# TencentYoutuResearch/NeRF-Loc

Measured on AMD Instinct MI355X. Metric: rendered rays/sec (4096 rays×128 samples, 256-wide MLP) at 1/2/4/8 MI355X, higher is better.
Workload: dtype f16mx (neural-point kernel, conv_out and feat_mlp.0: fp16 hi.hi + two MX-FP6 cross terms, 1.5 MFMA-equivalents per product; every other GEMM 3-term split-bf16 or split-fp16; fp32 accumulate; meets 1e-4)

## Files before the change

### nerf_loc_amd/csrc/hier.hip

```cpp
#include "mvdec.h"

namespace {
using namespace nlmv;

struct QueryCam { float w2c[12]; float kinv[9]; };

__global__ __launch_bounds__(256) void coarse_view_kernel(const NlViews vw, const QueryCam qc, const float* __restrict__ visf,
                                                          const float* __restrict__ dw, const float* __restrict__ pix ,
                                                          const float* __restrict__ zc , int R, int Sc,
                                                          float* __restrict__ alpha_out , float* __restrict__ vis_out,
                                                          float* __restrict__ mask_out) {
  const int i = blockIdx.x * blockDim.x + threadIdx.x;
  const int v = blockIdx.y;
  if (i >= R * Sc) return;
  const int r = i / Sc, s = i - r * Sc;
  const float u = pix[2 * r], vv = pix[2 * r + 1];
  const float* K = qc.kinv;
  const float c0 = K[0] * u + K[1] * vv + K[2], c1 = K[3] * u + K[4] * vv + K[5], c2 = K[6] * u + K[7] * vv + K[8];
  const float* Wm = qc.w2c;
  const float t0 = Wm[3], t1 = Wm[7], t2 = Wm[11];
  float cen[3], dir[3];
#pragma unroll
  for (int a = 0; a < 3; ++a) {
    const float r0 = Wm[a], r1 = Wm[4 + a], r2 = Wm[8 + a];
// ... 112 lines not shown
    al = al * (1.f - inv) + inv * -15.f;
    a = nl_sigmoid(al);
  }
  float inc = on ? 1.f - a : 1.f;
#pragma unroll
  for (int o = 1; o < 64; o <<= 1) {
    float t = __shfl_up(inc, o, 64);
    if (lane >= o) inc *= t;
  }
  float T = __shfl_up(inc, 1, 64);
  if (lane == 0) T = 1.f;
  const float w = on ? a * T : 0.f;
  if (on) weights[(size_t)r * Sc + lane] = w;
  const float d = wave_sum(on ? w * zc[(size_t)r * Sc + lane] : 0.f);
  if (lane == 0 && depth_coarse) depth_coarse[r] = d;
}

__global__ __launch_bounds__(256) void sample_pdf_kernel(const float* __restrict__ zc, const float* __restrict__ wc, int Sc,
                                                         const float* __restrict__ u, int Ni, const float* __restrict__ zb, int Sb,
                                                         int R, float* __restrict__ z_out) {
  __shared__ float s_cdf[4][64];
  __shared__ float s_bins[4][64];
  __shared__ float s_sort[4][256];
  const int lane = threadIdx.x & 63, wv = threadIdx.x >> 6;
  const int r = blockIdx.x * 4 + wv;
  if (r >= R) return;
  const int nb = Sc - 2;
  const float eps = 1e-5f;
  float wgt = (lane < nb) ? wc[(size_t)r * Sc + 1 + lane] + eps : 0.f;
  const float tot = wave_sum(wgt);
  const float pdf = wgt / tot;
  s_bins[wv][lane] = (lane < Sc - 1) ? 0.5f * (zc[(size_t)r * Sc + lane] + zc[(size_t)r * Sc + lane + 1]) : 0.f;
  s_cdf[wv][lane] = pdf;
  __builtin_amdgcn_wave_barrier();
  if (lane == 0) {
    float run = 0.f;
    float prev = 0.f;
    for (int i = 0; i < nb; ++i) { const float p = s_cdf[wv][i]; s_cdf[wv][i] = prev; run += p; prev = run; }
    s_cdf[wv][nb] = prev;
  }
  __builtin_amdgcn_wave_barrier();
  const int S = Sb + Ni;
  for (int i = lane; i < 256; i += 64) s_sort[wv][i] = i < Sb ? zb[(size_t)r * Sb + i] : 3.4e38f;
  for (int i = lane; i < Ni; i += 64) {
    const float uu = u[(size_t)r * Ni + i];
    int lo = 0, hi = nb + 1;
    while (lo < hi) { const int mid = (lo + hi) >> 1; if (s_cdf[wv][mid] > uu) hi = mid; else lo = mid + 1; }
    const int below = lo - 1 < 0 ? 0 : lo - 1;
    const int above = lo > nb ? nb : lo;
    const float c0 = s_cdf[wv][below], c1 = s_cdf[wv][above];
    const float b0 = s_bins[wv][below], b1 = s_bins[wv][above];
    float den = c1 - c0;
    if (den < eps) den = 1.f;
    s_sort[wv][Sb + i] = b0 + (uu - c0) / den * (b1 - b0);
  }
  __builtin_amdgcn_wave_barrier();
  for (int k = 2; k <= 256; k <<= 1) {
    for (int j = k >> 1; j > 0; j >>= 1) {
#pragma unroll
      for (int e = 0; e < 2; ++e) {
        const int t = lane + 64 * e;
        const int i = 2 * j * (t / j) + (t % j);
        const int p = i + j;
        const bool up = ((i & k) == 0);
        const float x = s_sort[wv][i], y = s_sort[wv][p];
        if ((x > y) == up) { s_sort[wv][i] = y; s_sort[wv][p] = x; }
      }
      __builtin_amdgcn_wave_barrier();
    }
  }
  for (int i = lane; i < S; i += 64) z_out[(size_t)r * S + i] = s_sort[wv][i];
}

}

int nl_launch_coarse_weights(const NlViews& vw, const float* w2c_kinv_host, const float* visf_hwc, const float* dec_w, const void* dpack,
                             int precision, const float* pix, const float* zc, int64_t R, int Sc, float* ws_alpha, float* ws_vis, float* ws_mask,
                             float* weights, float* depth_coarse, hipStream_t st) {
  if (R <= 0) return NL_OK;
  if (Sc < 3 || Sc > 64) return NL_ERR_UNSUPPORTED;
  QueryCam qc;
  for (int i = 0; i < 12; ++i) qc.w2c[i] = w2c_kinv_host[i];
  for (int i = 0; i < 9; ++i) qc.kinv[i] = w2c_kinv_host[12 + i];
  if (precision == NL_PREC_F32 || R * Sc > 0x7fffffffll / 32) {
    dim3 grid((unsigned)nl_cdiv(R * Sc, 256), (unsigned)vw.V);
    hipLaunchKernelGGL(coarse_view_kernel, grid, dim3(256), 0, st, vw, qc, visf_hwc, dec_w, pix, zc, (int)R, Sc, ws_alpha, ws_vis, ws_mask);
  } else {
    const int tpv = (int)nl_cdiv(R * Sc, 32), total = tpv * vw.V;
    const int blocks = (int)(nl_cdiv(total, 4) < 2048 ? nl_cdiv(total, 4) : 2048);
    hipLaunchKernelGGL(coarse_view_mfma_kernel<true>, dim3(blocks), dim3(256), 0, st, vw, qc, visf_hwc, (const uint4*)dpack, pix, zc, (int)R, Sc, tpv,
                       total, ws_alpha, ws_vis, ws_mask);
  }
  hipLaunchKernelGGL(coarse_ray_kernel, dim3((unsigned)nl_cdiv(R, 4)), dim3(256), 0, st, ws_alpha, ws_vis, ws_mask, zc, vw.V, (int)R, Sc,
                     weights, depth_coarse);
  NL_LAUNCH_CHECK();
  return NL_OK;
}

int nl_launch_sample_pdf(const float* zc, const float* wc, int Sc, const float* u, int Ni, const float* zb, int Sb, int64_t R,
                         float* z_out, hipStream_t st) {
  if (R <= 0) return NL_OK;
  if (Sc < 3 || Sc > 64 || Sb + Ni > 256 || Ni < 1) return NL_ERR_UNSUPPORTED;
  hipLaunchKernelGGL(sample_pdf_kernel, dim3((unsigned)nl_cdiv(R, 4)), dim3(256), 0, st, zc, wc, Sc, u, Ni, zb, Sb, (int)R, z_out);
  NL_LAUNCH_CHECK();
  return NL_OK;
}
```

### nerf_loc_amd/csrc/mvagg.hip

```cpp
#include "mvdec.h"

namespace {
using namespace nlmv;

__global__ void chw_to_hwc_kernel(const float* __restrict__ src, float* __restrict__ dst, int V, int Cc, int HW) {
  size_t i = (size_t)blockIdx.x * blockDim.x + threadIdx.x;
  size_t total = (size_t)V * Cc * HW;
  if (i >= total) return;
  int c = (int)(i % Cc);
  size_t t = i / Cc;
  int p = (int)(t % HW);
  int v = (int)(t / HW);
  dst[i] = src[((size_t)v * Cc + c) * HW + p];
}

__global__ __launch_bounds__(256) void mv_vis_kernel(const NlViews vw, const float* __restrict__ visf ,
                                                     const float* __restrict__ dw, const float* __restrict__ xyz, int N,
                                                     float* __restrict__ vis_out , float* __restrict__ dd_out ) {
  const int n = blockIdx.x * blockDim.x + threadIdx.x;
  const int v = blockIdx.y;
  if (n >= N) return;
  const float X = xyz[3 * (size_t)n], Y = xyz[3 * (size_t)n + 1], Z = xyz[3 * (size_t)n + 2];
  float px, py, depth;
  const bool valid = project_neuray(vw.P2[v], X, Y, Z, vw.Wimg, vw.H, px, py, depth);
  float x[32];
  sample_visf(visf + (size_t)v * vw.vh * vw.vw * 32, vw.vh, vw.vw, vw.Wimg, vw.H, px, py, valid, x);
  float m0, m1, v0, v1, aw, vs;
  decode_all(dw, x, m0, m1, v0, v1, vs, aw);

  const float ni = -1.f / vw.near_, fi = -1.f / vw.far_;
  float refd = -1.f / (m0 * (fi - ni) + ni);
  refd = fminf(fmaxf(refd, vw.near_), vw.far_);
  const float dd = fabsf(depth - refd) / (vw.far_ - vw.near_);
  const float dn = (-1.f / fmaxf(depth, 1e-5f) - ni) / (fi - ni);
  const float c0 = (0.5f + 0.5f * tanhf((dn - m0) * v0)) * vs;
  const float c1 = (0.5f + 0.5f * tanhf((dn - m1) * v1)) * vs;
  float vis = (1.f - c0) * aw + (1.f - c1) * (1.f - aw);
  vis = valid ? vis : 0.f;
  vis_out[(size_t)v * N + n] = vis;
  dd_out[(size_t)v * N + n] = dd;
}

template <bool X3>
__global__ __launch_bounds__(256) void mv_vis_mfma_kernel(const NlViews vw, const float* __restrict__ visf ,
                                                          const uint4* __restrict__ dpack, const float* __restrict__ xyz, int N,
                                                          int tiles_per_view, int total_tiles, float* __restrict__ vis_out,
                                                          float* __restrict__ dd_out) {
  __shared__ uint4 sw[MVD_LDS_UINT4];
  const int tid = threadIdx.x, lane = tid & 63, wave = tid >> 6;
  const int hh = lane >> 5, j = lane & 31;
  if (X3) __builtin_amdgcn_s_setreg(1473, 1);
  mvd_load_lds<X3>(sw, dpack, tid, 256);
  __syncthreads();

  for (int tile = blockIdx.x * 4 + wave; tile < total_tiles; tile += gridDim.x * 4) {
    const int v = __builtin_amdgcn_readfirstlane(tile / tiles_per_view);
    const int n = (tile - v * tiles_per_view) * 32 + j;
    const bool live = n < N;
    const int nn = live ? n : N - 1;
    const float X = xyz[3 * (size_t)nn], Y = xyz[3 * (size_t)nn + 1], Z = xyz[3 * (size_t)nn + 2];
    float px, py, depth;
    const bool valid = project_neuray(vw.P2[v], X, Y, Z, vw.Wimg, vw.H, px, py, depth);
    if (__ballot(valid && live) == 0ull) {
      if (live && hh == 0) {
        vis_out[(size_t)v * N + n] = 0.f;
        dd_out[(size_t)v * N + n] = 0.f;
      }
      continue;
    }
    float x0[8], x1[8];
    mvd_tap16(visf + (size_t)v * vw.vh * vw.vw * 32 + 8 * hh, vw.vh, vw.vw, vw.Wimg, vw.H, px, py, valid, x0, x1);
    float m0, m1, v0, v1, aw, vs;
    mvd_decode_tile<X3>(sw, lane, x0, x1, m0, m1, v0, v1, vs, aw);
    const float ni = -1.f / vw.near_, fi = -1.f / vw.far_;
    float refd = -1.f / (m0 * (fi - ni) + ni);
    refd = fminf(fmaxf(refd, vw.near_), vw.far_);
    const float dd = fabsf(depth - refd) / (vw.far_ - vw.near_);
    const float dn = (-1.f / fmaxf(depth, 1e-5f) - ni) / (fi - ni);
    const float c0 = (0.5f + 0.5f * tanhf((dn - m0) * v0)) * vs;
    const float c1 = (0.5f + 0.5f * tanhf((dn - m1) * v1)) * vs;
    float vis = (1.f - c0) * aw + (1.f - c1) * (1.f - aw);
    vis = valid ? vis : 0.f;
    if (live && hh == 0) {
      vis_out[(size_t)v * N + n] = vis;
      dd_out[(size_t)v * N + n] = dd;
    }
  }
}

__global__ void pack_mv_decoder_kernel(const float* __restrict__ dec , uint4* __restrict__ out) {
  unsigned short* o16 = reinterpret_cast<unsigned short*>(out);
  unsigned short* h16 = reinterpret_cast<unsigned short*>(out + MVD_F16);
  float* of = reinterpret_cast<float*>(out + MVD_F32);
  const int i = blockIdx.x * blockDim.x + threadIdx.x;
  auto f2bf = [](float x) { unsigned int u = __float_as_uint(x); u += 0x7fffu + ((u >> 16) & 1u); return (unsigned short)(u >> 16); };
  auto f2h = [](float x) { const _Float16 h = (_Float16)x; return __builtin_bit_cast(unsigned short, h); };
  auto h2f = [](unsigned short b) { return (float)__builtin_bit_cast(_Float16, b); };
  if (i < 4096) {
    const int t = i & 7, lane = (i >> 3) & 63, d = (i >> 9) & 3, q = i >> 11;
    const float v = dec[d * DEC_STRIDE + (lane & 31) * 32 + 16 * q + 8 * (lane >> 5) + t];
    const unsigned short h = f2bf(v);
    o16[(size_t)MVD_W1 * 8 + i] = h;
    o16[(size_t)(MVD_W1 + 512) * 8 + i] = f2bf(v - __uint_as_float(((unsigned)h) << 16));
    const unsigned short g = f2h(v);
    h16[(size_t)MVD_W1 * 8 + i] = g;
    h16[(size_t)(MVD_W1 + 512) * 8 + i] = f2h(v - h2f(g));
  } else if (i < 8192) {
    const int e = i - 4096;
    const int t = e & 7, lane = (e >> 3) & 63, s = (e >> 9) & 1, d = e >> 10;
    const int fin = 16 * s + (t & 3) + 8 * (t >> 2) + 4 * (lane >> 5);
    const float v = dec[d * DEC_STRIDE + 1056 + (lane & 31) * 32 + fin];
    const unsigned short h = f2bf(v);
    o16[(size_t)MVD_W2 * 8 + e] = h;
    o16[(size_t)(MVD_W2 + 512) * 8 + e] = f2bf(v - __uint_as_float(((unsigned)h) << 16));
    const unsigned short g = f2h(v);
    h16[(size_t)MVD_W2 * 8 + e] = g;
    h16[(size_t)(MVD_W2 + 512) * 8 + e] = f2h(v - h2f(g));
  } else if (i < 8192 + 128) { const int e = i - 8192; of[e] = dec[(e >> 5) * DEC_STRIDE + 1024 + (e & 31)]; }
  else if (i < 8192 + 256) { const int e = i - 8192 - 128; of[128 + e] = dec[(e >> 5) * DEC_STRIDE + 2080 + (e & 31)]; }
  else if (i < 8192 + 512) {
    const int e = i - 8192 - 256;
    const int r = e & 15, hh = (e >> 4) & 1, u = (e >> 5) & 1, d = e >> 6;
    const int idx = (r & 3) + 8 * (r >> 2) + 4 * hh;
    of[256 + e] = dec[d * DEC_STRIDE + 2112 + u * 32 + idx];
  } else if (i < 8192 + 520) { const int e = i - 8192 - 512; of[512 + e] = dec[(e >> 1) * DEC_STRIDE + 2176 + (e & 1)]; }
  if (i < 8192) {
    unsigned short* t16 = reinterpret_cast<unsigned short*>(out + MVD_T);
    const int which = i >> 12, e = i & 4095;
    const int t = e & 7, lane = (e >> 3) & 63, s = (e >> 9) & 1, d = e >> 10;
    const int u = 16 * s + (t & 3) + 8 * (t >> 2) + 4 * (lane >> 5);
    const int row = lane & 31;
    float v;
    if (which == 0) v = dec[d * DEC_STRIDE + 1056 + u * 32 + row];
    else {
      const int hh = (row >> 2) & 1, r = (row & 3) + 4 * (row >> 3);
      const int chan = r < 8 ? 8 * hh + r : 16 + 8 * hh + (r - 8);
      v = dec[d * DEC_STRIDE + u * 32 + chan];
    }
    const unsigned short h = f2bf(v);
    t16[(size_t)which * 1024 * 8 + e] = h;
    t16[(size_t)which * 1024 * 8 + 512 * 8 + e] = f2bf(v - __uint_as_float(((unsigned)h) << 16));
  }
}

__device__ __forceinline__ float rl(float v, int lane) { return __int_as_float(__builtin_amdgcn_readlane(__float_as_int(v), lane)); }
__device__ __forceinline__ int rli(int v, int lane) { return __builtin_amdgcn_readlane(v, lane); }

template <int VT, bool V4, bool EXACT>
__global__ __launch_bounds__(256, VT <= 4 ? 4 : (VT <= 10 ? 3 : 2)) void mv_stats_kernel(const NlViews vw, const float* __restrict__ viewsdev ,
                                                       const float* __restrict__ images ,
                                                       const float* __restrict__ feat , int C,
                                                       const float* __restrict__ xyz, int N,
                                                       const float* __restrict__ vis_in, const float* __restrict__ dd_in,
                                                       float* __restrict__ g393, int ldg, float* __restrict__ rgb_feat ,
                                                       float* __restrict__ vis_ang , int* __restrict__ valid_s,
                                                       const float* __restrict__ pfeat ,
                                                       const float* __restrict__ blw ,
                                                       float* __restrict__ bl1 , float* __restrict__ rgbv ) {
  const int lane = threadIdx.x & 63;
  const int n = nl_xcd_block() * 4 + (threadIdx.x >> 6);
  if (n >= N) return;
  const int V = EXACT ? VT : vw.V;
  const float X = xyz[3 * (size_t)n], Y = xyz[3 * (size_t)n + 1], Z = xyz[3 * (size_t)n + 2];
  const int F = C + 3;

  const int vl = lane < V ? lane : 0;
// ... 357 lines not shown
    Tap4 cur = issue(0);
#pragma unroll
    for (int v = 0; v < VT; ++v) {
      if (v < V) {
        Tap4 nxt = cur;
        if (v + 1 < VT && v + 1 < V) nxt = issue(v + 1);
        if (!active(v)) {
          if (live) {
            *(float4*)(bl1 + ((size_t)n * V + v) * 32 + 4 * j) = make_float4(0.f, 0.f, 0.f, 0.f);
            if (j == 0) *(float4*)(rgbv + ((size_t)n * V + v) * 4) = make_float4(slot0[v * MS8_SLOT + 17], slot0[v * MS8_SLOT + 18], slot0[v * MS8_SLOT + 19], 0.f);
          }
          cur = nxt;
          continue;
        }
        const float* sl = slot0 + v * MS8_SLOT;
        const float4 w = *(const float4*)(sl + 2), ang = *(const float4*)(sl + 10);
        const float s_vis = sl[14], r = sl[17], gg = sl[18], b = sl[19];
        const float pv[4] = {fmaf(cur.t[3].x, w.w, fmaf(cur.t[2].x, w.z, fmaf(cur.t[1].x, w.y, cur.t[0].x * w.x))),
                             fmaf(cur.t[3].y, w.w, fmaf(cur.t[2].y, w.z, fmaf(cur.t[1].y, w.y, cur.t[0].y * w.x))),
                             fmaf(cur.t[3].z, w.w, fmaf(cur.t[2].z, w.z, fmaf(cur.t[1].z, w.y, cur.t[0].z * w.x))),
                             fmaf(cur.t[3].w, w.w, fmaf(cur.t[2].w, w.z, fmaf(cur.t[1].w, w.y, cur.t[0].w * w.x)))};
        float o[4];
#pragma unroll
        for (int c = 0; c < 4; ++c) {
          float a = pv[c] + bb[c];
          a = fmaf(bw[c][0], r, a); a = fmaf(bw[c][1], gg, a); a = fmaf(bw[c][2], b, a);
          a = fmaf(bw[c][3], s_vis, a);
          a = fmaf(bw[c][4], ang.x, a); a = fmaf(bw[c][5], ang.y, a); a = fmaf(bw[c][6], ang.z, a); a = fmaf(bw[c][7], ang.w, a);
          o[c] = a;
        }
        if (live) {
          *(float4*)(bl1 + ((size_t)n * V + v) * 32 + 4 * j) = make_float4(o[0], o[1], o[2], o[3]);
          if (j == 0) *(float4*)(rgbv + ((size_t)n * V + v) * 4) = make_float4(r, gg, b, s_vis);
        }
        cur = nxt;
      }
    }
  }

  if (live && j == 0) {
    float mean = 0.f, wsum = 0.f;
#pragma unroll
    for (int v = 0; v < VT; ++v) { if (v < V) { mean += slot0[v * MS8_SLOT + 15] * wg[v]; wsum += wg[v]; } }
    float var = 0.f;
#pragma unroll
    for (int v = 0; v < VT; ++v) { if (v < V) { const float d = slot0[v * MS8_SLOT + 15] - mean; var += wg[v] * (d * d); } }
    g[2 * F] = mean;
    g[2 * F + 1] = var;
    g[2 * F + 2] = wsum / (float)V;
    for (int p = 2 * F + 3; p < ldg; ++p) g[p] = 0.f;
    valid_s[n] = cnt1 > 1 ? 1 : 0;
  }
}

}

int nl_launch_chw_to_hwc(const float* src, float* dst, int V, int Cc, int HW, hipStream_t st) {
  size_t total = (size_t)V * Cc * HW;
  hipLaunchKernelGGL(chw_to_hwc_kernel, dim3((unsigned)nl_cdiv(total, 256)), dim3(256), 0, st, src, dst, V, Cc, HW);
  NL_LAUNCH_CHECK();
  return NL_OK;
}

int nl_launch_mv_vis(const NlViews& vw, const float* visf_hwc, const float* dec_w, const float* xyz, int64_t N,
                     float* vis_out, float* dd_out, hipStream_t st) {
  if (N <= 0) return NL_OK;
  dim3 grid((unsigned)nl_cdiv(N, 256), (unsigned)vw.V);
  hipLaunchKernelGGL(mv_vis_kernel, grid, dim3(256), 0, st, vw, visf_hwc, dec_w, xyz, (int)N, vis_out, dd_out);
  NL_LAUNCH_CHECK();
  return NL_OK;
}

size_t nl_mv_decoder_pack_bytes() { return (size_t)MVD_PACK_UINT4 * 16; }

int nl_pack_mv_decoder(const float* dec_valu_layout, void* out, hipStream_t st) {
  hipLaunchKernelGGL(pack_mv_decoder_kernel, dim3((8192 + 520 + 255) / 256), dim3(256), 0, st, dec_valu_layout, (uint4*)out);
  NL_LAUNCH_CHECK();
  return NL_OK;
}

int nl_launch_mv_vis_mfma(const NlViews& vw, const float* visf_hwc, const void* dpack, const float* xyz, int64_t N, float* vis_out,
                          float* dd_out, bool x3, hipStream_t st) {
  if (N <= 0) return NL_OK;
  const int tpv = (int)nl_cdiv(N, 32), total = tpv * vw.V;
  constexpr int64_t max_blocks = 2048;
  const int blocks = (int)(nl_cdiv(total, 4) < max_blocks ? nl_cdiv(total, 4) : max_blocks);
  if (x3) hipLaunchKernelGGL(mv_vis_mfma_kernel<true>, dim3(blocks), dim3(256), 0, st, vw, visf_hwc, (const uint4*)dpack, xyz, (int)N, tpv, total, vis_out, dd_out);
  else hipLaunchKernelGGL(mv_vis_mfma_kernel<false>, dim3(blocks), dim3(256), 0, st, vw, visf_hwc, (const uint4*)dpack, xyz, (int)N, tpv, total, vis_out, dd_out);
  NL_LAUNCH_CHECK();
  return NL_OK;
}

int nl_launch_mv_stats(const NlViews& vw, const float* viewsdev, const float* images, const float* feat, int C, const float* xyz, int64_t N,
                       const float* vis_in, const float* dd_in, float* g393, int ldg, float* rgb_feat, float* vis_ang,
                       int* valid_s, const float* pfeat, const float* blw, float* bl1, float* rgbv, hipStream_t st) {
  if (N <= 0) return NL_OK;
  if (C > 192) return NL_ERR_UNSUPPORTED;
  const bool v4 = (C % 4 == 0) && ((((size_t)feat) & 15) == 0);
  if (v4 && !rgb_feat && !vis_ang) {
    dim3 grid8(nl_xcd_grid(nl_cdiv(N, 32)));
#define NL_MS8(VT) hipLaunchKernelGGL((mv_stats8_kernel<VT>), grid8, dim3(256), sizeof(float) * 4 * 8 * VT * MS8_SLOT, st, vw, viewsdev, images, feat, C, \
                                      xyz, (int)N, vis_in, dd_in, g393, ldg, valid_s, pfeat, blw, bl1, rgbv)
    if (vw.V <= 4) NL_MS8(4); else if (vw.V <= 8) NL_MS8(8); else if (vw.V <= 10) NL_MS8(10); else NL_MS8(16);
#undef NL_MS8
    NL_LAUNCH_CHECK();
    return NL_OK;
  }
  dim3 grid(nl_xcd_grid(nl_cdiv(N, 4)));
  const bool ex = vw.V == 4 || vw.V == 8 || vw.V == 10 || vw.V == 16;
#define NL_MS1(VT, V4, EX)                                                                                                              \
  hipLaunchKernelGGL((mv_stats_kernel<VT, V4, EX>), grid, dim3(256), 0, st, vw, viewsdev, images, feat, C, xyz, (int)N, vis_in, dd_in, \
                     g393, ldg, rgb_feat, vis_ang, valid_s, pfeat, blw, bl1, rgbv)
#define NL_MS1_BUCKET(VT)                 \
  do {                                    \
    if (v4 && ex) NL_MS1(VT, true, true); \
    else if (v4) NL_MS1(VT, true, false); \
    else NL_MS1(VT, false, false);        \
  } while (0)
  if (vw.V <= 4) NL_MS1_BUCKET(4);
  else if (vw.V <= 8) NL_MS1_BUCKET(8);
  else if (vw.V <= 10) NL_MS1_BUCKET(10);
  else NL_MS1_BUCKET(16);
#undef NL_MS1_BUCKET
#undef NL_MS1
  NL_LAUNCH_CHECK();
  return NL_OK;
}
```

### nerf_loc_amd/csrc/mvdec.h

```cpp
#pragma once
#include "common.h"

namespace nlmv {

struct Taps {
  int x0, y0;
  float nw, ne, sw, se;
  bool mw, me, mn, ms;
};

template <bool ALIGN, bool BORDER>
__device__ __forceinline__ Taps make_taps(float xn, float yn, int Wm, int Hm) {
  float ix, iy;
  if (ALIGN) {
    ix = (xn + 1.f) * ((float)(Wm - 1) / 2.f);
    iy = (yn + 1.f) * ((float)(Hm - 1) / 2.f);
  } else {
    ix = (xn + 1.f) * ((float)Wm / 2.f) - 0.5f;
    iy = (yn + 1.f) * ((float)Hm / 2.f) - 0.5f;
  }
  if (BORDER) {
    ix = fminf((float)(Wm - 1), fmaxf(ix, 0.f));
    iy = fminf((float)(Hm - 1), fmaxf(iy, 0.f));
  }
// ... 44 lines not shown
  const float* w4 = w2 + 1024 + 32;
  float a0 = w4[64], a1 = w4[65];
#pragma unroll
  for (int i = 0; i < 32; ++i) {
    a0 = fmaf(w4[i], h2[i], a0);
    a1 = fmaf(w4[32 + i], h2[i], a1);
  }
  o0 = a0;
  o1 = a1;
}


__device__ __forceinline__ bool project_neuray(const float* P, float X, float Y, float Z, int Wimg, int H, float& px, float& py, float& depth) {
  const float cx = fmaf(P[2], Z, fmaf(P[1], Y, P[0] * X)) + P[3];
  const float cy = fmaf(P[6], Z, fmaf(P[5], Y, P[4] * X)) + P[7];
  depth = fmaf(P[10], Z, fmaf(P[9], Y, P[8] * X)) + P[11];
  const bool bad = fabsf(depth) < 1e-4f;
  if (bad) depth = 1e-3f;
  px = cx / depth; py = cy / depth;
  const bool outside = (px < -0.5f) | (px >= (float)Wimg - 0.5f) | (py < -0.5f) | (py >= (float)H - 0.5f);
  return !bad && !outside;
}

__device__ __forceinline__ void sample_visf(const float* __restrict__ base, int h, int w, int Wimg, int H, float px, float py, bool valid, float (&x)[32]) {
  if (valid) {
    const float xn = px / (float)(Wimg - 1) * 2.f - 1.f;
    const float yn = py / (float)(H - 1) * 2.f - 1.f;
    const Taps t = make_taps<false, true>(xn, yn, w, h);
    const int xe = t.x0 + 1, ys = t.y0 + 1;
#pragma unroll
    for (int c4 = 0; c4 < 8; ++c4) {
      float4 a = make_float4(0, 0, 0, 0), b = a, c = a, d = a;
      if (t.mn && t.mw) a = *(const float4*)(base + ((size_t)t.y0 * w + t.x0) * 32 + c4 * 4);
      if (t.mn && t.me) b = *(const float4*)(base + ((size_t)t.y0 * w + xe) * 32 + c4 * 4);
      if (t.ms && t.mw) c = *(const float4*)(base + ((size_t)ys * w + t.x0) * 32 + c4 * 4);
      if (t.ms && t.me) d = *(const float4*)(base + ((size_t)ys * w + xe) * 32 + c4 * 4);
      x[c4 * 4 + 0] = a.x * t.nw + b.x * t.ne + c.x * t.sw + d.x * t.se;
      x[c4 * 4 + 1] = a.y * t.nw + b.y * t.ne + c.y * t.sw + d.y * t.se;
      x[c4 * 4 + 2] = a.z * t.nw + b.z * t.ne + c.z * t.sw + d.z * t.se;
      x[c4 * 4 + 3] = a.w * t.nw + b.w * t.ne + c.w * t.sw + d.w * t.se;
    }
  } else {
#pragma unroll
    for (int i = 0; i < 32; ++i) x[i] = 0.f;
  }
}

__device__ __forceinline__ void decode_all(const float* __restrict__ dw, const float (&x)[32], float& m0, float& m1, float& v0, float& v1, float& vs, float& aw) {
  float dummy;
  decoder(dw + 0 * DEC_STRIDE, x, m0, m1);
  decoder(dw + 1 * DEC_STRIDE, x, v0, v1);
  decoder(dw + 2 * DEC_STRIDE, x, aw, dummy);
  decoder(dw + 3 * DEC_STRIDE, x, vs, dummy);
  m0 = nl_softplus(m0); m1 = nl_softplus(m1);
  v0 = nl_softplus(v0) + 0.05f; v1 = nl_softplus(v1) + 0.05f;
  aw = nl_sigmoid(aw); vs = nl_sigmoid(vs);
}

typedef __bf16 mvd_bf16x8 __attribute__((ext_vector_type(8)));
typedef _Float16 mvd_f16x8 __attribute__((ext_vector_type(8)));
typedef float mvd_f32x16 __attribute__((ext_vector_type(16)));

constexpr int MVD_W1 = 0;
constexpr int MVD_W2 = 1024;
constexpr int MVD_F32 = 2048;
constexpr int MVD_NF32 = (128 + 128 + 256 + 8) / 4;
constexpr int MVD_F16 = MVD_F32 + MVD_NF32;
constexpr int MVD_T = MVD_F16 + 2048;
constexpr int MVD_PACK_UINT4 = MVD_T + 2048;
constexpr int MVD_LDS_UINT4 = 2048 + MVD_NF32;

template <bool X3>
__device__ __forceinline__ void mvd_load_lds(uint4* sw, const uint4* __restrict__ dpack, int tid, int nthreads) {
  for (int i = tid; i < 2048; i += nthreads) sw[i] = dpack[(X3 ? MVD_F16 : 0) + i];
  for (int i = tid; i < MVD_NF32; i += nthreads) sw[2048 + i] = dpack[MVD_F32 + i];
}

template <bool X3> struct MvdOps;
typedef unsigned mvd_u32x4 __attribute__((ext_vector_type(4)));
template <> struct MvdOps<true> {
  typedef mvd_f16x8 v8;
  static __device__ __forceinline__ void split(const float (&v)[8], v8& hi, v8& lo) {
    mvd_u32x4 h, l;
#pragma unroll
    for (int t = 0; t < 4; ++t) {
      unsigned hp, lp; float l0, l1;
      asm("v_cvt_pk_f16_f32 %0, %3, %4\n\tv_fma_mix_f32 %1, %0, -1.0, %3 op_sel_hi:[1,0,0]\n\tv_fma_mix_f32 %2, %0, -1.0, %4 op_sel:[1,0,0] op_sel_hi:[1,0,0]"
          : "=&v"(hp), "=&v"(l0), "=&v"(l1) : "v"(v[2 * t]), "v"(v[2 * t + 1]));
      asm("v_cvt_pk_f16_f32 %0, %1, %2" : "=v"(lp) : "v"(l0), "v"(l1));
      h[t] = hp; l[t] = lp;
    }
    hi = __builtin_bit_cast(v8, h); lo = __builtin_bit_cast(v8, l);
  }
  static __device__ __forceinline__ mvd_f32x16 mfma(v8 a, v8 b, mvd_f32x16 c) { return __builtin_amdgcn_mfma_f32_32x32x16_f16(a, b, c, 0, 0, 0); }
};
template <> struct MvdOps<false> {
  typedef mvd_bf16x8 v8;
  static __device__ __forceinline__ void split(const float (&v)[8], v8& hi, v8& lo) {
#pragma unroll
    for (int t = 0; t < 8; ++t) hi[t] = (__bf16)v[t];
    lo = hi;
  }
  static __device__ __forceinline__ mvd_f32x16 mfma(v8 a, v8 b, mvd_f32x16 c) { return __builtin_amdgcn_mfma_f32_32x32x16_bf16(a, b, c, 0, 0, 0); }
};

__device__ __forceinline__ void mvd_split_bf16(const float (&v)[8], mvd_bf16x8& hi, mvd_bf16x8& lo) {
#pragma unroll
  for (int t = 0; t < 8; ++t) { const __bf16 h = (__bf16)v[t]; hi[t] = h; lo[t] = (__bf16)(v[t] - (float)h); }
}

typedef float mvd_f32x2 __attribute__((ext_vector_type(2)));
__device__ __forceinline__ void mvd_elu2(float& a, float& b) {
  const mvd_f32x2 x = {a, b};
  const mvd_f32x2 y = x * mvd_f32x2{1.4426950408889634f, 1.4426950408889634f};
  mvd_f32x2 e = {__builtin_amdgcn_exp2f(y[0]), __builtin_amdgcn_exp2f(y[1])};
  e = e - mvd_f32x2{1.f, 1.f};
  a = __builtin_amdgcn_fmed3f(x[0], e[0], 0.f);
  b = __builtin_amdgcn_fmed3f(x[1], e[1], 0.f);
}

__device__ __forceinline__ void mvd_tap16(const float* __restrict__ base , int vh, int vw_, int Wimg, int H, float px, float py,
                                          bool valid, float (&x0)[8], float (&x1)[8]) {
  const float xn = px / (float)(Wimg - 1) * 2.f - 1.f;
  const float yn = py / (float)(H - 1) * 2.f - 1.f;
  const Taps t = make_taps<false, true>(xn, yn, vw_, vh);
  const size_t o00 = ((size_t)(t.mn ? t.y0 : 0) * vw_ + (t.mw ? t.x0 : 0)) * 32;
  const size_t o01 = ((size_t)(t.mn ? t.y0 : 0) * vw_ + (t.me ? t.x0 + 1 : 0)) * 32;
  const size_t o10 = ((size_t)(t.ms ? t.y0 + 1 : 0) * vw_ + (t.mw ? t.x0 : 0)) * 32;
  const size_t o11 = ((size_t)(t.ms ? t.y0 + 1 : 0) * vw_ + (t.me ? t.x0 + 1 : 0)) * 32;
  const float w00 = (valid && t.mn && t.mw) ? t.nw : 0.f, w01 = (valid && t.mn && t.me) ? t.ne : 0.f;
  const float w10 = (valid && t.ms && t.mw) ? t.sw : 0.f, w11 = (valid && t.ms && t.me) ? t.se : 0.f;
#pragma unroll
  for (int g = 0; g < 2; ++g) {
#pragma unroll
    for (int c4 = 0; c4 < 2; ++c4) {
      const int co = 16 * g + 4 * c4;
      const float4 a = *(const float4*)(base + o00 + co), b = *(const float4*)(base + o01 + co);
      const float4 c = *(const float4*)(base + o10 + co), d = *(const float4*)(base + o11 + co);
      float* dst = g ? x1 : x0;
      dst[4 * c4 + 0] = fmaf(d.x, w11, fmaf(c.x, w10, fmaf(b.x, w01, a.x * w00)));
      dst[4 * c4 + 1] = fmaf(d.y, w11, fmaf(c.y, w10, fmaf(b.y, w01, a.y * w00)));
      dst[4 * c4 + 2] = fmaf(d.z, w11, fmaf(c.z, w10, fmaf(b.z, w01, a.z * w00)));
      dst[4 * c4 + 3] = fmaf(d.w, w11, fmaf(c.w, w10, fmaf(b.w, w01, a.w * w00)));
    }
  }
}

template <bool X3>
__device__ __forceinline__ void mvd_decode_tile(const uint4* sw, int lane, const float (&x0)[8], const float (&x1)[8], float& m0, float& m1,
                                                float& v0, float& v1, float& vs, float& aw) {
  typedef MvdOps<X3> OP;
  typedef typename OP::v8 v8;
  const int hh = lane >> 5;
  const float* sf = reinterpret_cast<const float*>(sw + 2048);
  const float* b1 = sf, *b2 = sf + 128, *w4p = sf + 256, *b4 = sf + 512;
  v8 xh[2], xl[2];
  OP::split(x0, xh[0], xl[0]);
  OP::split(x1, xh[1], xl[1]);
  float o[4][2];
#pragma unroll
  for (int d = 0; d < 4; ++d) {
    mvd_f32x16 acc;
#pragma unroll
    for (int g = 0; g < 4; ++g) {
      const float4 b = *(const float4*)(b1 + 32 * d + 8 * g + 4 * hh);
      acc[4 * g] = b.x; acc[4 * g + 1] = b.y; acc[4 * g + 2] = b.z; acc[4 * g + 3] = b.w;
    }
#pragma unroll
    for (int q = 0; q < 2; ++q) {
      const v8 ah = __builtin_bit_cast(v8, sw[MVD_W1 + (q * 4 + d) * 64 + lane]);
      if (X3) {
        const v8 al = __builtin_bit_cast(v8, sw[MVD_W1 + 512 + (q * 4 + d) * 64 + lane]);
        acc = OP::mfma(al, xh[q], acc);
        acc = OP::mfma(ah, xl[q], acc);
      }
      acc = OP::mfma(ah, xh[q], acc);
    }
    v8 gh[2], gl[2];
#pragma unroll
    for (int s = 0; s < 2; ++s) {
      float vv[8];
#pragma unroll
      for (int t = 0; t < 8; ++t) vv[t] = acc[8 * s + t];
#pragma unroll
      for (int t = 0; t < 8; t += 2) mvd_elu2(vv[t], vv[t + 1]);
      OP::split(vv, gh[s], gl[s]);
    }
    mvd_f32x16 acc2;
#pragma unroll
    for (int g = 0; g < 4; ++g) {
      const float4 b = *(const float4*)(b2 + 32 * d + 8 * g + 4 * hh);
      acc2[4 * g] = b.x; acc2[4 * g + 1] = b.y; acc2[4 * g + 2] = b.z; acc2[4 * g + 3] = b.w;
    }
#pragma unroll
    for (int s = 0; s < 2; ++s) {
      const v8 ah = __builtin_bit_cast(v8, sw[MVD_W2 + (d * 2 + s) * 64 + lane]);
      if (X3) {
        const v8 al = __builtin_bit_cast(v8, sw[MVD_W2 + 512 + (d * 2 + s) * 64 + lane]);
        acc2 = OP::mfma(al, gh[s], acc2);
        acc2 = OP::mfma(ah, gl[s], acc2);
      }
      acc2 = OP::mfma(ah, gh[s], acc2);
    }
    float h2[16];
#pragma unroll
    for (int r = 0; r < 16; ++r) h2[r] = acc2[r];
#pragma unroll
    for (int r = 0; r < 16; r += 2) mvd_elu2(h2[r], h2[r + 1]);
#pragma unroll
    for (int u = 0; u < 2; ++u) {
      float p = 0.f;
      if (u == 0 || d < 2) {
        const float* w = w4p + ((d * 2 + u) * 2 + hh) * 16;
#pragma unroll
        for (int r4 = 0; r4 < 4; ++r4) {
          const float4 ww = *(const float4*)(w + 4 * r4);
          p = fmaf(ww.x, h2[4 * r4], p); p = fmaf(ww.y, h2[4 * r4 + 1], p);
          p = fmaf(ww.z, h2[4 * r4 + 2], p); p = fmaf(ww.w, h2[4 * r4 + 3], p);
        }
        p += __shfl_xor(p, 32, 64);
        p += b4[d * 2 + u];
      }
      o[d][u] = p;
    }
  }
  m0 = nl_softplus(o[0][0]); m1 = nl_softplus(o[0][1]);
  v0 = nl_softplus(o[1][0]) + 0.05f; v1 = nl_softplus(o[1][1]) + 0.05f;
  aw = nl_sigmoid(o[2][0]); vs = nl_sigmoid(o[3][0]);
}

}
```

Before: 584,900.

## Process two 32-point tiles per wave in visibility decoder with lane-swapped taps

The MFMA visibility kernel now has each wave cover a pair of 32-point tiles: both half-waves project their own points, and tap offsets and weights are exchanged with permlane32_swap so the whole wave decodes each tile in turn. Before, the second half-wave did redundant projection and never wrote results. Tile offsets move to 32-bit (guarded by a new map-size check that falls back to the scalar path), ELU and the fp16 split are batched into wider instruction groups, and waves-per-EU hints are added. Costs are more registers for the two tap sets, plus a serial decode loop that only skips a tile when none of its points are valid.

```diff
diff --git a/nerf_loc_amd/csrc/hier.hip b/nerf_loc_amd/csrc/hier.hip
--- a/nerf_loc_amd/csrc/hier.hip
+++ b/nerf_loc_amd/csrc/hier.hip
@@ -218,7 +218,7 @@
   QueryCam qc;
   for (int i = 0; i < 12; ++i) qc.w2c[i] = w2c_kinv_host[i];
   for (int i = 0; i < 9; ++i) qc.kinv[i] = w2c_kinv_host[12 + i];
-  if (precision == NL_PREC_F32 || R * Sc > 0x7fffffffll / 32) {
+  if (precision == NL_PREC_F32 || R * Sc > 0x7fffffffll / 32 || !nlmv::mvd_map_fits(vw.vh, vw.vw)) {
     dim3 grid((unsigned)nl_cdiv(R * Sc, 256), (unsigned)vw.V);
     hipLaunchKernelGGL(coarse_view_kernel, grid, dim3(256), 0, st, vw, qc, visf_hwc, dec_w, pix, zc, (int)R, Sc, ws_alpha, ws_vis, ws_mask);
   } else {
diff --git a/nerf_loc_amd/csrc/mvagg.hip b/nerf_loc_amd/csrc/mvagg.hip
--- a/nerf_loc_amd/csrc/mvagg.hip
+++ b/nerf_loc_amd/csrc/mvagg.hip
@@ -42,10 +42,9 @@
 }
 
 template <bool X3>
-__global__ __launch_bounds__(256) void mv_vis_mfma_kernel(const NlViews vw, const float* __restrict__ visf ,
-                                                          const uint4* __restrict__ dpack, const float* __restrict__ xyz, int N,
-                                                          int tiles_per_view, int total_tiles, float* __restrict__ vis_out,
-                                                          float* __restrict__ dd_out) {
+__global__ __launch_bounds__(256) __attribute__((amdgpu_waves_per_eu(X3 ? 4 : 1, X3 ? 4 : 8)))
+void mv_vis_mfma_kernel(const NlViews vw, const float* __restrict__ visf , const uint4* __restrict__ dpack, const float* __restrict__ xyz,
+                        int N, int pairs_per_view, int total_pairs, float* __restrict__ vis_out, float* __restrict__ dd_out) {
   __shared__ uint4 sw[MVD_LDS_UINT4];
   const int tid = threadIdx.x, lane = tid & 63, wave = tid >> 6;
   const int hh = lane >> 5, j = lane & 31;
@@ -53,35 +52,51 @@
   mvd_load_lds<X3>(sw, dpack, tid, 256);
   __syncthreads();
 
-  for (int tile = blockIdx.x * 4 + wave; tile < total_tiles; tile += gridDim.x * 4) {
-    const int v = __builtin_amdgcn_readfirstlane(tile / tiles_per_view);
-    const int n = (tile - v * tiles_per_view) * 32 + j;
+  for (int pair = blockIdx.x * 4 + wave; pair < total_pairs; pair += gridDim.x * 4) {
+    const int v = __builtin_amdgcn_readfirstlane(pair / pairs_per_view);
+    const int n = ((pair - v * pairs_per_view) * 2 + hh) * 32 + j;
     const bool live = n < N;
     const int nn = live ? n : N - 1;
     const float X = xyz[3 * (size_t)nn], Y = xyz[3 * (size_t)nn + 1], Z = xyz[3 * (size_t)nn + 2];
     float px, py, depth;
     const bool valid = project_neuray(vw.P2[v], X, Y, Z, vw.Wimg, vw.H, px, py, depth);
-    if (__ballot(valid && live) == 0ull) {
-      if (live && hh == 0) {
-        vis_out[(size_t)v * N + n] = 0.f;
-        dd_out[(size_t)v * N + n] = 0.f;
-      }
-      continue;
-    }
-    float x0[8], x1[8];
-    mvd_tap16(visf + (size_t)v * vw.vh * vw.vw * 32 + 8 * hh, vw.vh, vw.vw, vw.Wimg, vw.H, px, py, valid, x0, x1);
+    const unsigned long long seen = __ballot(valid && live);
+    const bool on[2] = {(unsigned)seen != 0u, (unsigned)(seen >> 32) != 0u};
+    float o[6] = {0.f, 0.f, 0.f, 0.f, 0.f, 0.f};
+    if (seen != 0ull) {
+      const MvdTap own = mvd_tap_setup(vw.vh, vw.vw, vw.Wimg, vw.H, px, py, valid);
+      MvdTap tp[2];
+#pragma unroll
+      for (int k = 0; k < 4; ++k) {
+        const auto ro = __builtin_amdgcn_permlane32_swap(own.o[k], own.o[k], false, false);
+        const auto rw = __builtin_amdgcn_permlane32_swap(__float_as_uint(own.w[k]), __float_as_uint(own.w[k]), false, false);
+        tp[0].o[k] = ro[0]; tp[1].o[k] = ro[1];
+        tp[0].w[k] = __uint_as_float(rw[0]); tp[1].w[k] = __uint_as_float(rw[1]);
+      }
+      const float* vbase = visf + (size_t)v * vw.vh * vw.vw * 32 + 8 * hh;
+#pragma unroll
+      for (int t = 0; t < 2; ++t) {
+        if (!on[t]) continue;
+        float x0[8], x1[8], r[6];
+        mvd_tap_fetch(vbase, tp[t], x0, x1);
+        mvd_decode_raw<X3>(sw, lane, x0, x1, r);
+#pragma unroll
+        for (int k = 0; k < 6; ++k) o[k] = hh == t ? r[k] : o[k];
+      }
+    }
     float m0, m1, v0, v1, aw, vs;
-    mvd_decode_tile<X3>(sw, lane, x0, x1, m0, m1, v0, v1, vs, aw);
+    mvd_decode_act(o, m0, m1, v0, v1, vs, aw);
     const float ni = -1.f / vw.near_, fi = -1.f / vw.far_;
     float refd = -1.f / (m0 * (fi - ni) + ni);
     refd = fminf(fmaxf(refd, vw.near_), vw.far_);
-    const float dd = fabsf(depth - refd) / (vw.far_ - vw.near_);
+    float dd = fabsf(depth - refd) / (vw.far_ - vw.near_);
     const float dn = (-1.f / fmaxf(depth, 1e-5f) - ni) / (fi - ni);
     const float c0 = (0.5f + 0.5f * tanhf((dn - m0) * v0)) * vs;
     const float c1 = (0.5f + 0.5f * tanhf((dn - m1) * v1)) * vs;
     float vis = (1.f - c0) * aw + (1.f - c1) * (1.f - aw);
     vis = valid ? vis : 0.f;
-    if (live && hh == 0) {
+    dd = on[hh] ? dd : 0.f;
+    if (live) {
       vis_out[(size_t)v * N + n] = vis;
       dd_out[(size_t)v * N + n] = dd;
     }
@@ -605,11 +620,12 @@
 int nl_launch_mv_vis_mfma(const NlViews& vw, const float* visf_hwc, const void* dpack, const float* xyz, int64_t N, float* vis_out,
                           float* dd_out, bool x3, hipStream_t st) {
   if (N <= 0) return NL_OK;
-  const int tpv = (int)nl_cdiv(N, 32), total = tpv * vw.V;
+  if (!mvd_map_fits(vw.vh, vw.vw)) return NL_ERR_UNSUPPORTED;
+  const int ppv = (int)nl_cdiv(nl_cdiv(N, 32), 2), total = ppv * vw.V;
   constexpr int64_t max_blocks = 2048;
   const int blocks = (int)(nl_cdiv(total, 4) < max_blocks ? nl_cdiv(total, 4) : max_blocks);
-  if (x3) hipLaunchKernelGGL(mv_vis_mfma_kernel<true>, dim3(blocks), dim3(256), 0, st, vw, visf_hwc, (const uint4*)dpack, xyz, (int)N, tpv, total, vis_out, dd_out);
-  else hipLaunchKernelGGL(mv_vis_mfma_kernel<false>, dim3(blocks), dim3(256), 0, st, vw, visf_hwc, (const uint4*)dpack, xyz, (int)N, tpv, total, vis_out, dd_out);
+  if (x3) hipLaunchKernelGGL(mv_vis_mfma_kernel<true>, dim3(blocks), dim3(256), 0, st, vw, visf_hwc, (const uint4*)dpack, xyz, (int)N, ppv, total, vis_out, dd_out);
+  else hipLaunchKernelGGL(mv_vis_mfma_kernel<false>, dim3(blocks), dim3(256), 0, st, vw, visf_hwc, (const uint4*)dpack, xyz, (int)N, ppv, total, vis_out, dd_out);
   NL_LAUNCH_CHECK();
   return NL_OK;
 }
diff --git a/nerf_loc_amd/csrc/mvdec.h b/nerf_loc_amd/csrc/mvdec.h
--- a/nerf_loc_amd/csrc/mvdec.h
+++ b/nerf_loc_amd/csrc/mvdec.h
@@ -150,14 +150,18 @@
   typedef mvd_f16x8 v8;
   static __device__ __forceinline__ void split(const float (&v)[8], v8& hi, v8& lo) {
     mvd_u32x4 h, l;
-#pragma unroll
-    for (int t = 0; t < 4; ++t) {
-      unsigned hp, lp; float l0, l1;
-      asm("v_cvt_pk_f16_f32 %0, %3, %4\n\tv_fma_mix_f32 %1, %0, -1.0, %3 op_sel_hi:[1,0,0]\n\tv_fma_mix_f32 %2, %0, -1.0, %4 op_sel:[1,0,0] op_sel_hi:[1,0,0]"
-          : "=&v"(hp), "=&v"(l0), "=&v"(l1) : "v"(v[2 * t]), "v"(v[2 * t + 1]));
-      asm("v_cvt_pk_f16_f32 %0, %1, %2" : "=v"(lp) : "v"(l0), "v"(l1));
-      h[t] = hp; l[t] = lp;
-    }
+    unsigned h0, h1, h2, h3, p0, p1, p2, p3;
+    float q0, q1, q2, q3;
+    asm("v_cvt_pk_f16_f32 %0, %12, %13\n\tv_cvt_pk_f16_f32 %1, %14, %15\n\tv_cvt_pk_f16_f32 %2, %16, %17\n\tv_cvt_pk_f16_f32 %3, %18, %19\n\t"
+        "v_fma_mix_f32 %4, %0, -1.0, %12 op_sel_hi:[1,0,0]\n\tv_fma_mix_f32 %8, %0, -1.0, %13 op_sel:[1,0,0] op_sel_hi:[1,0,0]\n\t"
+        "v_fma_mix_f32 %5, %1, -1.0, %14 op_sel_hi:[1,0,0]\n\tv_fma_mix_f32 %9, %1, -1.0, %15 op_sel:[1,0,0] op_sel_hi:[1,0,0]\n\t"
+        "v_fma_mix_f32 %6, %2, -1.0, %16 op_sel_hi:[1,0,0]\n\tv_fma_mix_f32 %10, %2, -1.0, %17 op_sel:[1,0,0] op_sel_hi:[1,0,0]\n\t"
+        "v_fma_mix_f32 %7, %3, -1.0, %18 op_sel_hi:[1,0,0]\n\tv_fma_mix_f32 %11, %3, -1.0, %19 op_sel:[1,0,0] op_sel_hi:[1,0,0]\n\t"
+        "v_cvt_pk_f16_f32 %4, %4, %8\n\tv_cvt_pk_f16_f32 %5, %5, %9\n\tv_cvt_pk_f16_f32 %6, %6, %10\n\tv_cvt_pk_f16_f32 %7, %7, %11"
+        : "=&v"(h0), "=&v"(h1), "=&v"(h2), "=&v"(h3), "=&v"(p0), "=&v"(p1), "=&v"(p2), "=&v"(p3), "=&v"(q0), "=&v"(q1), "=&v"(q2), "=&v"(q3)
+        : "v"(v[0]), "v"(v[1]), "v"(v[2]), "v"(v[3]), "v"(v[4]), "v"(v[5]), "v"(v[6]), "v"(v[7]));
+    h[0] = h0; h[1] = h1; h[2] = h2; h[3] = h3;
+    l[0] = p0; l[1] = p1; l[2] = p2; l[3] = p3;
     hi = __builtin_bit_cast(v8, h); lo = __builtin_bit_cast(v8, l);
   }
   static __device__ __forceinline__ mvd_f32x16 mfma(v8 a, v8 b, mvd_f32x16 c) { return __builtin_amdgcn_mfma_f32_32x32x16_f16(a, b, c, 0, 0, 0); }
@@ -178,45 +182,61 @@
 }
 
 typedef float mvd_f32x2 __attribute__((ext_vector_type(2)));
-__device__ __forceinline__ void mvd_elu2(float& a, float& b) {
-  const mvd_f32x2 x = {a, b};
-  const mvd_f32x2 y = x * mvd_f32x2{1.4426950408889634f, 1.4426950408889634f};
-  mvd_f32x2 e = {__builtin_amdgcn_exp2f(y[0]), __builtin_amdgcn_exp2f(y[1])};
-  e = e - mvd_f32x2{1.f, 1.f};
-  a = __builtin_amdgcn_fmed3f(x[0], e[0], 0.f);
-  b = __builtin_amdgcn_fmed3f(x[1], e[1], 0.f);
-}
-
-__device__ __forceinline__ void mvd_tap16(const float* __restrict__ base , int vh, int vw_, int Wimg, int H, float px, float py,
-                                          bool valid, float (&x0)[8], float (&x1)[8]) {
+__device__ __forceinline__ void mvd_elu8(float (&v)[8]) {
+  const mvd_f32x2 k = {1.4426950408889634f, 1.4426950408889634f};
+  mvd_f32x2 x[4], y[4], e[4];
+#pragma unroll
+  for (int p = 0; p < 4; ++p) { x[p] = mvd_f32x2{v[2 * p], v[2 * p + 1]}; y[p] = x[p] * k; }
+#pragma unroll
+  for (int p = 0; p < 4; ++p) e[p] = mvd_f32x2{__builtin_amdgcn_exp2f(y[p][0]), __builtin_amdgcn_exp2f(y[p][1])};
+#pragma unroll
+  for (int p = 0; p < 4; ++p) e[p] = e[p] - mvd_f32x2{1.f, 1.f};
+#pragma unroll
+  for (int p = 0; p < 4; ++p) {
+    v[2 * p] = __builtin_amdgcn_fmed3f(x[p][0], e[p][0], 0.f);
+    v[2 * p + 1] = __builtin_amdgcn_fmed3f(x[p][1], e[p][1], 0.f);
+  }
+}
+
+struct MvdTap { unsigned o[4]; float w[4]; };
+inline bool mvd_map_fits(int vh, int vw_) { return (unsigned long long)vh * (unsigned long long)vw_ * 32ull < (1ull << 32); }
+__device__ __forceinline__ MvdTap mvd_tap_setup(int vh, int vw_, int Wimg, int H, float px, float py, bool valid) {
   const float xn = px / (float)(Wimg - 1) * 2.f - 1.f;
   const float yn = py / (float)(H - 1) * 2.f - 1.f;
   const Taps t = make_taps<false, true>(xn, yn, vw_, vh);
-  const size_t o00 = ((size_t)(t.mn ? t.y0 : 0) * vw_ + (t.mw ? t.x0 : 0)) * 32;
-  const size_t o01 = ((size_t)(t.mn ? t.y0 : 0) * vw_ + (t.me ? t.x0 + 1 : 0)) * 32;
-  const size_t o10 = ((size_t)(t.ms ? t.y0 + 1 : 0) * vw_ + (t.mw ? t.x0 : 0)) * 32;
-  const size_t o11 = ((size_t)(t.ms ? t.y0 + 1 : 0) * vw_ + (t.me ? t.x0 + 1 : 0)) * 32;
-  const float w00 = (valid && t.mn && t.mw) ? t.nw : 0.f, w01 = (valid && t.mn && t.me) ? t.ne : 0.f;
-  const float w10 = (valid && t.ms && t.mw) ? t.sw : 0.f, w11 = (valid && t.ms && t.me) ? t.se : 0.f;
+  MvdTap m;
+  m.o[0] = ((unsigned)(t.mn ? t.y0 : 0) * vw_ + (t.mw ? t.x0 : 0)) * 32;
+  m.o[1] = ((unsigned)(t.mn ? t.y0 : 0) * vw_ + (t.me ? t.x0 + 1 : 0)) * 32;
+  m.o[2] = ((unsigned)(t.ms ? t.y0 + 1 : 0) * vw_ + (t.mw ? t.x0 : 0)) * 32;
+  m.o[3] = ((unsigned)(t.ms ? t.y0 + 1 : 0) * vw_ + (t.me ? t.x0 + 1 : 0)) * 32;
+  m.w[0] = (valid && t.mn && t.mw) ? t.nw : 0.f; m.w[1] = (valid && t.mn && t.me) ? t.ne : 0.f;
+  m.w[2] = (valid && t.ms && t.mw) ? t.sw : 0.f; m.w[3] = (valid && t.ms && t.me) ? t.se : 0.f;
+  return m;
+}
+__device__ __forceinline__ void mvd_tap_fetch(const float* __restrict__ base , const MvdTap& m, float (&x0)[8], float (&x1)[8]) {
 #pragma unroll
   for (int g = 0; g < 2; ++g) {
 #pragma unroll
     for (int c4 = 0; c4 < 2; ++c4) {
       const int co = 16 * g + 4 * c4;
-      const float4 a = *(const float4*)(base + o00 + co), b = *(const float4*)(base + o01 + co);
-      const float4 c = *(const float4*)(base + o10 + co), d = *(const float4*)(base + o11 + co);
+      const float4 a = *(const float4*)(base + m.o[0] + co), b = *(const float4*)(base + m.o[1] + co);
+      const float4 c = *(const float4*)(base + m.o[2] + co), d = *(const float4*)(base + m.o[3] + co);
       float* dst = g ? x1 : x0;
-      dst[4 * c4 + 0] = fmaf(d.x, w11, fmaf(c.x, w10, fmaf(b.x, w01, a.x * w00)));
-      dst[4 * c4 + 1] = fmaf(d.y, w11, fmaf(c.y, w10, fmaf(b.y, w01, a.y * w00)));
-      dst[4 * c4 + 2] = fmaf(d.z, w11, fmaf(c.z, w10, fmaf(b.z, w01, a.z * w00)));
-      dst[4 * c4 + 3] = fmaf(d.w, w11, fmaf(c.w, w10, fmaf(b.w, w01, a.w * w00)));
-    }
-  }
+      dst[4 * c4 + 0] = fmaf(d.x, m.w[3], fmaf(c.x, m.w[2], fmaf(b.x, m.w[1], a.x * m.w[0])));
+      dst[4 * c4 + 1] = fmaf(d.y, m.w[3], fmaf(c.y, m.w[2], fmaf(b.y, m.w[1], a.y * m.w[0])));
+      dst[4 * c4 + 2] = fmaf(d.z, m.w[3], fmaf(c.z, m.w[2], fmaf(b.z, m.w[1], a.z * m.w[0])));
+      dst[4 * c4 + 3] = fmaf(d.w, m.w[3], fmaf(c.w, m.w[2], fmaf(b.w, m.w[1], a.w * m.w[0])));
+    }
+  }
+}
+__device__ __forceinline__ void mvd_tap16(const float* __restrict__ base , int vh, int vw_, int Wimg, int H, float px, float py,
+                                          bool valid, float (&x0)[8], float (&x1)[8]) {
+  const MvdTap m = mvd_tap_setup(vh, vw_, Wimg, H, px, py, valid);
+  mvd_tap_fetch(base, m, x0, x1);
 }
 
 template <bool X3>
-__device__ __forceinline__ void mvd_decode_tile(const uint4* sw, int lane, const float (&x0)[8], const float (&x1)[8], float& m0, float& m1,
-                                                float& v0, float& v1, float& vs, float& aw) {
+__device__ __forceinline__ void mvd_decode_raw(const uint4* sw, int lane, const float (&x0)[8], const float (&x1)[8], float (&out)[6]) {
   typedef MvdOps<X3> OP;
   typedef typename OP::v8 v8;
   const int hh = lane >> 5;
@@ -250,8 +270,7 @@
       float vv[8];
 #pragma unroll
       for (int t = 0; t < 8; ++t) vv[t] = acc[8 * s + t];
-#pragma unroll
-      for (int t = 0; t < 8; t += 2) mvd_elu2(vv[t], vv[t + 1]);
+      mvd_elu8(vv);
       OP::split(vv, gh[s], gl[s]);
     }
     mvd_f32x16 acc2;
@@ -272,9 +291,15 @@
     }
     float h2[16];
 #pragma unroll
-    for (int r = 0; r < 16; ++r) h2[r] = acc2[r];
-#pragma unroll
-    for (int r = 0; r < 16; r += 2) mvd_elu2(h2[r], h2[r + 1]);
+    for (int s = 0; s < 2; ++s) {
+      float vv[8];
+#pragma unroll
+      for (int t = 0; t < 8; ++t) vv[t] = acc2[8 * s + t];
+      mvd_elu8(vv);
+      asm("" : "+v"(vv[0]), "+v"(vv[1]), "+v"(vv[2]), "+v"(vv[3]), "+v"(vv[4]), "+v"(vv[5]), "+v"(vv[6]), "+v"(vv[7]));
+#pragma unroll
+      for (int t = 0; t < 8; ++t) h2[8 * s + t] = vv[t];
+    }
 #pragma unroll
     for (int u = 0; u < 2; ++u) {
       float p = 0.f;
@@ -292,9 +317,19 @@
       o[d][u] = p;
     }
   }
-  m0 = nl_softplus(o[0][0]); m1 = nl_softplus(o[0][1]);
-  v0 = nl_softplus(o[1][0]) + 0.05f; v1 = nl_softplus(o[1][1]) + 0.05f;
-  aw = nl_sigmoid(o[2][0]); vs = nl_sigmoid(o[3][0]);
-}
-
-}
+  out[0] = o[0][0]; out[1] = o[0][1]; out[2] = o[1][0]; out[3] = o[1][1]; out[4] = o[2][0]; out[5] = o[3][0];
+}
+__device__ __forceinline__ void mvd_decode_act(const float (&o)[6], float& m0, float& m1, float& v0, float& v1, float& vs, float& aw) {
+  m0 = nl_softplus(o[0]); m1 = nl_softplus(o[1]);
+  v0 = nl_softplus(o[2]) + 0.05f; v1 = nl_softplus(o[3]) + 0.05f;
+  aw = nl_sigmoid(o[4]); vs = nl_sigmoid(o[5]);
+}
+template <bool X3>
+__device__ __forceinline__ void mvd_decode_tile(const uint4* sw, int lane, const float (&x0)[8], const float (&x1)[8], float& m0, float& m1,
+                                                float& v0, float& v1, float& vs, float& aw) {
+  float o[6];
+  mvd_decode_raw<X3>(sw, lane, x0, x1, o);
+  mvd_decode_act(o, m0, m1, v0, v1, vs, aw);
+}
+
+}
```

Result: faster. 593,400, median of 6 (+1.5%).
